# Charrrrrlie/X-as-Supervision

Hardware: AMD Instinct MI355X
Metric: images/sec HM36_Multi_SurS1 256px bs32 (full disc+gen training step) (higher is better)
Workload: dtype f32 (f16x3 split: every fp32 operand as two fp16 pieces, three products; f32 accumulate); 1 GPU; HM36_Multi_SurS1; batch_per_gpu=32, cameras=4, image=256x256, parallelism=dp1, ranks=1, precision=f16x3, dedupe=False, full=False

## Files before the change

include/xas_hip.h:

```cpp
#ifndef XAS_HIP_H
#define XAS_HIP_H

#include <stddef.h>
#include <stdint.h>

#ifdef __cplusplus
extern "C" {
#endif

const char* xas_last_error(void);
enum {
  XAS_TUNE_WGRAD_SPLIT_XCD = 1,
  XAS_TUNE_PLAIN_KLOOP = 32,
  XAS_TUNE_GLOBAL_LOAD = 64,
  XAS_TUNE_WGRAD_GLOBAL_LOAD = 128,
  XAS_TUNE_WGRAD_ALT_ORDER = 8192,
  XAS_TUNE_WGRAD_PLAIN_KLOOP = 524288,
  XAS_TUNE_SLAB_SHIFT = 15,
  XAS_TUNE_SLAB_MASK = 3,
  XAS_TUNE_SLAB_512 = 32768,
  XAS_TUNE_SLAB_128 = 65536,
  XAS_TUNE_SLAB_64 = 98304,
  XAS_TUNE_COL_REDUCE_LEAN = 262144,
  XAS_TUNE_GENERAL_KERNELS = 1 << 22,
  XAS_TUNE_NO_WIDE_TILES = 1 << 23,
  XAS_TUNE_NO_STEM_WGRAD = 1 << 24,
  XAS_TUNE_STEM_FWD_F32 = 1 << 25,
  XAS_TUNE_NO_X6P = 1 << 26,
  XAS_TUNE_X6P_ANY_K = 1 << 27
};
int xas_set_tuning(int flags);
enum { XAS_PREC_F32 = 0, XAS_PREC_BF16 = 1, XAS_PREC_BF16X6 = 2, XAS_PREC_F16X3 = 3 };
#define XAS_AMAX_SUB 32
#define XAS_AMAX_STRIDE 32
#define XAS_AMAX_SLOT_FLOATS (XAS_AMAX_SUB * XAS_AMAX_STRIDE)
enum { XAS_GRAD_IS_X = 0x100 };
int xas_set_precision(int mode);
int xas_get_precision(void);
int xas_abi_version(void);

#define XAS_HEAD_STATS 16
size_t xas_head_workspace_floats(int B, int K, int D);
int xas_head_softargmax_fwd(const float* logits, int B, int K, int D, int num_hypo, int neighbor,
                            float* kps, int64_t* z_idx, float* depth_prob_map, int groups, float* stats,
                            float* partial, void* stream);
int xas_head_softargmax_from_partials(const float* partial, int B, int K, int D, int nchunk, int num_hypo, int neighbor,
                                      float* kps, int64_t* z_idx, float* depth_prob_map, int groups, float* stats,
                                      void* stream);

int xas_head_softargmax_bwd(const float* logits, const float* stats, const int64_t* z_idx,
                            const float* grad_kps, int B, int K, int D, int num_hypo, int neighbor,
                            float* grad_logits, float* coef, void* stream);
int xas_head_softargmax_bwd_amax(const float* logits, const float* stats, const int64_t* z_idx,
                                 const float* grad_kps, int B, int K, int D, int num_hypo, int neighbor,
                                 float* grad_logits, float* coef, float* amax_out, void* stream);

#define XAS_GEO_NORM 1
#define XAS_GEO_MONO 2
#define XAS_GEO_PATCH 4
#define XAS_GEO_IMAGE 8
int xas_patch_to_world_fwd(const float* kps, const float* trans_image, const float* k_mat,
                           const float* pelvis, const float* rot_world, const float* trans_world,
                           int B, int Hy, int K, float image_size, float rect_width, int flags,
                           float* world, void* stream);
int xas_patch_to_world_bwd(const float* kps, const float* grad_world, const float* trans_image,
                           const float* k_mat, const float* pelvis, const float* rot_world,
                           const float* trans_world, int B, int Hy, int K, float image_size,
                           float rect_width, int flags, float* grad_kps, void* stream);

#define XAS_GEO_WORLD 16
int xas_world_to_patch_fwd(const float* pts, const float* pre_rot, float pre_scale, int pelvis_origin,
                           const float* trans_image, const float* k_mat, const float* pelvis,
                           const float* rot_world, const float* trans_world, int B, int Hy, int K,
                           float image_size, float rect_width, int flags, float* out, void* stream);
int xas_world_to_patch_bwd(const float* pts, const float* grad_out, const float* pre_rot, float pre_scale,
                           int pelvis_origin, const float* trans_image, const float* k_mat, const float* pelvis,
                           const float* rot_world, const float* trans_world, int B, int Hy, int K,
                           float image_size, float rect_width, int flags, float* grad_pts, float* grad_pre_rot,
                           void* stream);

int xas_lines_nblk(int S);
int xas_draw_lines_max_fwd(const float* kps, long kp_stride_b, long kp_stride_j, int B, int K,
                           const int* parents, const int* children, int L, unsigned fine_mask,
                           float body_width, int S, float* mask, void* stream);
int xas_draw_lines_max_bwd(const float* kps, long kp_stride_b, long kp_stride_j, int B, int K,
                           const int* parents, const int* children, int L, unsigned fine_mask,
                           float body_width, int S, const float* grad_mask, float* partial,
                           float* grad_kps_xy , void* stream);

typedef struct {
  int N, Hi, Wi, Cin;
  int Cout, R, S;
  int stride, pad;
  int Ho, Wo;
  int mode;
  const float* grad_amax;
  const float* x_amax;
} xas_conv_shape;

int xas_conv_weight_planes(const xas_conv_shape* s, int pass);
int xas_conv_kernel_class(const xas_conv_shape* s, int pass);
int xas_f16_weight_overflow(int reset);
int xas_f16_weight_overflow_peek(unsigned* device_out, void* stream);
size_t xas_split_weight_bytes(long rows, long K, int pieces);
int xas_split_weight(const float* w_packed, void* w_split, long rows, long K, int pieces, void* stream);

int xas_prepare_weights(const void* descs, int n, long blocks, void* stream);

int xas_conv_fwd(const float* x, const float* w_packed, const float* bias, float* y,
                 const xas_conv_shape* s, void* stream);

int xas_conv_fwd_head_chunks(const xas_conv_shape* s, int K, int D);
int xas_conv_fwd_head(const float* x, const float* w_packed, const float* bias, float* y, const xas_conv_shape* s,
                      int K, int D, float* head_partial, void* stream);
size_t xas_conv_fwd_bnstats_workspace_floats(const xas_conv_shape* s, int groups);
int xas_conv_fwd_bnstats(const float* x, const float* w_packed, float* y, const xas_conv_shape* s, int groups,
                         const float* pivot, float* mean, float* var_biased, long out_stride, float* count_out,
                         float* workspace, float* running_mean, float* running_var, float momentum, void* stream);
size_t xas_conv_dgrad_bn_bwd_workspace_floats(const xas_conv_shape* s, int groups);
int xas_conv_dgrad_bn_bwd(const float* dy, const float* w_packed_t, const xas_conv_shape* s, const float* xb,
                          const float* mean, const float* var_biased, const float* gamma, const float* beta, float eps,
                          int groups, double count, float* dz, float* dx, float* sums, float* workspace, float* dbeta_acc,
                          float* dgamma_acc, void* stream);
int xas_conv_dgrad(const float* dy, const float* w_packed_t, float* dx,
                   const xas_conv_shape* s, void* stream);
int xas_conv_dgrad_acc(const float* dy, const float* w_packed_t, float* dx, const xas_conv_shape* shape, void* stream);
int xas_conv_dgrad_acc_masked(const float* dy, const float* w_packed_t, float* dx, const xas_conv_shape* s,
                              const float* dprev, const uint8_t* mask, void* stream);
size_t xas_conv_wgrad_workspace_floats(const xas_conv_shape* s);
int xas_conv_wgrad(const float* x, const float* dy, float* dw_packed, float* workspace,
                   const xas_conv_shape* s, void* stream);
int xas_conv_wgrad_oihw(const float* x, const float* dy, float* dw_oihw, float* workspace,
                        const xas_conv_shape* s, void* stream);
int xas_conv_wgrad_acc(const float* x, const float* dy, float* dw_oihw, float* workspace,
                       const xas_conv_shape* s, void* stream);
int xas_pack_weight(const float* oihw, float* packed, int Cout, int Cin, int R, int S,
                    int transposed, void* stream);
int xas_unpack_weight(const float* packed, float* oihw, int Cout, int Cin, int R, int S,
// ... 128 lines not shown
```

x-as-supervision_amd/csrc/head.hip:

```cpp
#include "common.h"

namespace xas {

struct HeadGeom {
  int B, K, D, HW, W, C4, G, rec;
  int KT, ntile, C4t;
  int R, rh, rw, wshift;
  int P, nchunk;
};

static int pow2_slots(long C4) {
  int gcd = 1;
  while (gcd < 64 && (C4 % (gcd * 2)) == 0) gcd *= 2;
  return 64 / gcd;
}

static bool pow2_policy(int D, int K) {
  if (!(D >= 4 && D <= 64 && (D & (D - 1)) == 0) || (tune_flags() & XAS_TUNE_GENERAL_KERNELS)) return false;
  if (K <= 0) return true;
  const long C4 = (long)K * (D / 4);
  const int R = pow2_slots(C4);
  return R <= D * D && C4 * R <= 1024;
}

// ... 177 lines not shown
  }
  const float S = wave_sum(sd0 + sd1);
  const float pz0 = live0 ? sd0 / S : 0.f, pz1 = live1 ? sd1 / S : 0.f;
  const float X = SX / S, Y = SY / S;
  float* st = stats + ((size_t)b * g.K + k) * XAS_HEAD_STATS;
  if (b % dmap_every == 0) {
    float* dm = depth_prob_map + ((size_t)(b / dmap_every) * g.K + k) * g.D;
    if (live0) dm[d0] = pz0;
    if (live1) dm[d1] = pz1;
  }
  const float fD = (float)g.D;
  const float xn = X / fD * 2.f - 1.f, yn = Y / fD * 2.f - 1.f;
  if (lane == 0) { st[0] = M + __logf(S); st[1] = X; st[2] = Y; }

  if (neighbor == 0) {
    const float Z = wave_sum(pz0 * (float)d0 + pz1 * (float)d1);
    if (lane == 0) {
      float* o = kps + ((size_t)b * g.K + k) * 3;
      o[0] = xn; o[1] = yn; o[2] = Z / fD * 2.f - 1.f;
      st[3] = Z;
      if (z_idx) z_idx[(size_t)b * g.K + k] = 0;
    }
    return;
  }
  float left0 = __shfl_up(pz0, 1, 64), right0 = __shfl_down(pz0, 1, 64);
  float left1 = __shfl_up(pz1, 1, 64), right1 = __shfl_down(pz1, 1, 64);
  const float bin64 = __shfl(pz1, 0, 64), bin63 = __shfl(pz0, 63, 64);
  if (lane == 63) right0 = bin64;
  if (lane == 0) left1 = bin63;
  const bool inner0 = d0 >= 1 && d0 <= g.D - 2, inner1 = d1 <= g.D - 2;
  float score0 = inner0 ? ((pz0 >= left0 && pz0 >= right0) ? pz0 : 0.f) : -1.f;
  float score1 = inner1 ? ((pz1 >= left1 && pz1 >= right1) ? pz1 : 0.f) : -1.f;
  const int r = neighbor / 2;
  for (int h = 0; h < num_hypo; ++h) {
    const float best = wave_max(fmaxf(score0, score1));
    const unsigned long long cand0 = __ballot(score0 == best), cand1 = __ballot(score1 == best);
    const int idx = cand0 ? __ffsll((long long)cand0) - 1 : 64 + __ffsll((long long)cand1) - 1;
    if (d0 == idx) score0 = -2.f;
    if (d1 == idx) score1 = -2.f;
    const bool in0 = live0 && (d0 >= idx - r) && (d0 <= idx + r);
    const bool in1 = live1 && (d1 >= idx - r) && (d1 <= idx + r);
    const float sw = wave_sum((in0 ? pz0 : 0.f) + (in1 ? pz1 : 0.f));
    const float swd = wave_sum((in0 ? pz0 * (float)d0 : 0.f) + (in1 ? pz1 * (float)d1 : 0.f));
    const float Z = swd / sw;
    if (lane == 0) {
      float* o = kps + (((size_t)b * num_hypo + h) * g.K + k) * 3;
      o[0] = xn; o[1] = yn; o[2] = Z / fD * 2.f - 1.f;
      z_idx[((size_t)b * g.K + k) * num_hypo + h] = idx;
      st[3 + h] = Z;
      st[9 + h] = sw;
    }
  }
}

__global__ void head_bwd_coef_kernel(const float* __restrict__ stats, const int64_t* __restrict__ z_idx,
                                     const float* __restrict__ grad_kps, HeadGeom g, int num_hypo, int neighbor,
                                     float* __restrict__ coef) {
  const int b = blockIdx.x / g.K, k = blockIdx.x % g.K;
  const int d = threadIdx.x;
  const float* st = stats + ((size_t)b * g.K + k) * XAS_HEAD_STATS;
  const float fD = (float)g.D;
  float gx = 0.f, gy = 0.f, gz = 0.f, c0 = 0.f;
  const int r = neighbor / 2;
  for (int h = 0; h < num_hypo; ++h) {
    const float* gk = grad_kps + (((size_t)b * num_hypo + h) * g.K + k) * 3;
    gx += gk[0];
    gy += gk[1];
    if (neighbor == 0) {
      const float cz = gk[2] * (2.f / fD);
      gz += cz * (float)d;
      c0 -= cz * st[3];
    } else {
      const int idx = (int)z_idx[((size_t)b * g.K + k) * num_hypo + h];
      if (d >= idx - r && d <= idx + r) gz += gk[2] * (2.f / fD) * ((float)d - st[3 + h]) / st[9 + h];
    }
  }
  const float cx = gx * (2.f / fD), cy = gy * (2.f / fD);
  c0 += -cx * st[1] - cy * st[2];
  float* o = coef + ((size_t)b * g.K + k) * (4 + g.D);
  if (d == 0) { o[0] = cx; o[1] = cy; o[2] = c0; o[3] = st[0]; }
  if (d < g.D) o[4 + d] = gz;
}

template <bool POW2>
__global__ void head_bwd_kernel(const float4* __restrict__ logits, const float* __restrict__ coef, HeadGeom g,
                                float4* __restrict__ grad, float* __restrict__ amax_out) {
  __shared__ unsigned s_amax;
  if (threadIdx.x == 0) s_amax = 0u;
  if (amax_out) __syncthreads();
  float amx = 0.f;
  const int KT = POW2 ? g.K : g.KT, C4t = POW2 ? g.C4 : g.C4t;
  const int tid = threadIdx.x;
  const int c4t = tid % C4t, slot = tid / C4t;
  const int kt = c4t / g.G, dq = c4t % g.G;
  const int bz = POW2 ? 0 : blockIdx.z;
  const int k = bz * KT + kt;
  const int b = blockIdx.y, chunk = blockIdx.x;
  const int pix0 = chunk * g.P;
  const int pend = min(g.P, g.HW - pix0);
  if (POW2 || k < g.K) {
    const float* cf = coef + ((size_t)b * g.K + k) * (4 + g.D);
    const float cx = cf[0], cy = cf[1], c0 = cf[2], lse = cf[3];
    const float4 gz = *reinterpret_cast<const float4*>(cf + 4 + 4 * dq);
    const size_t off = ((size_t)b * g.HW + pix0) * g.C4 + (k * g.G + dq);
    PixelWalk<POW2> walk(g, pix0 + slot);
#pragma unroll 4
    for (int p = slot; p < pend; p += g.R) {
      const float4 v = stream_load(logits + off + (size_t)p * g.C4);
      float fh, fw;
      walk.next(g, pix0 + p, &fh, &fw);
      const float lin = cx * fw + cy * fh + c0;
      float4 o;
      o.x = __expf(v.x - lse) * (lin + gz.x);
      o.y = __expf(v.y - lse) * (lin + gz.y);
      o.z = __expf(v.z - lse) * (lin + gz.z);
      o.w = __expf(v.w - lse) * (lin + gz.w);
      amx = amax4(amx, o);
      stream_store(grad + off + (size_t)p * g.C4, o);
    }
  }
  if (amax_out) {
    if (amx > 0.f) atomicMax(&s_amax, __float_as_uint(amx));
    __syncthreads();
    const unsigned sub = (blockIdx.x + (blockIdx.y + bz * gridDim.y) * gridDim.x) % (unsigned)kAmaxSub;
    if (threadIdx.x == 0 && s_amax) atomicMax(reinterpret_cast<unsigned*>(amax_out + sub * kAmaxStride), s_amax);
  }
}

static int check_modes(const char* who, int D, int num_hypo, int neighbor, const int64_t* z_idx, int B, int groups) {
  XAS_REQUIRE(num_hypo >= 1 && num_hypo <= 6, "%s: num_hypo %d not in [1,6]", who, num_hypo);
  XAS_REQUIRE(neighbor >= 0 && (neighbor > 0 || num_hypo == 1), "%s: single-hypothesis mode needs num_hypo == 1", who);
  XAS_REQUIRE(neighbor == 0 || (z_idx != nullptr && num_hypo <= D - 2), "%s: z_idx required / too many hypotheses", who);
  XAS_REQUIRE(groups >= 1 && B % groups == 0, "%s: B=%d does not split into %d groups", who, B, groups);
  return 0;
}

static int check_grid(const char* who, const HeadGeom& g) {
  XAS_REQUIRE(g.B <= 65535 && g.ntile <= 65535, "%s: B=%d K=%d exceed the launch grid", who, g.B, g.K);
  return 0;
}

static int launch_finalize(const float* partial, const HeadGeom& g, int num_hypo, int neighbor, float* kps, int64_t* z_idx,
                           float* depth_prob_map, int groups, float* stats, void* stream) {
  hipLaunchKernelGGL(head_finalize_kernel, dim3(g.B * g.K), dim3(64), 0, as_stream(stream), partial, g, num_hypo,
                     neighbor, kps, z_idx, depth_prob_map, g.B / groups, stats);
  XAS_LAUNCH_CHECK();
  return 0;
}

}

using namespace xas;

extern "C" size_t xas_head_workspace_floats(int B, int K, int D) {
  HeadGeom g;
  if (make_geom(B, K, D, pow2_policy(D, K), &g)) return 0;
  return (size_t)B * g.nchunk * K * g.rec;
}

extern "C" int xas_head_softargmax_fwd(const float* logits, int B, int K, int D, int num_hypo, int neighbor,
                                       float* kps, int64_t* z_idx, float* depth_prob_map, int groups, float* stats,
                                       float* partial, void* stream) {
  const bool pow2 = pow2_policy(D, K);
  HeadGeom g;
  if (make_geom(B, K, D, pow2, &g)) return 1;
  XAS_REQUIRE(logits && kps && depth_prob_map && stats && partial, "head fwd: null buffer");
  if (check_modes("head fwd", D, num_hypo, neighbor, z_idx, B, groups)) return 1;
  XAS_REQUIRE(((uintptr_t)logits & 15) == 0, "head fwd: logits must be 16-byte aligned");
  const size_t lds = partial_lds_bytes(g, pow2);
  XAS_REQUIRE(lds <= 64 * 1024, "head fwd: LDS %zu too large", lds);
  if (check_grid("head fwd", g)) return 1;
  hipLaunchKernelGGL(pow2 ? head_partial_kernel<true> : head_partial_kernel<false>, dim3(g.nchunk, B, g.ntile),
                     dim3(g.C4t * g.R), lds, as_stream(stream), reinterpret_cast<const float4*>(logits), partial, g);
  XAS_LAUNCH_CHECK();
  return launch_finalize(partial, g, num_hypo, neighbor, kps, z_idx, depth_prob_map, groups, stats, stream);
}

extern "C" int xas_head_softargmax_from_partials(const float* partial, int B, int K, int D, int nchunk, int num_hypo, int neighbor,
                                                 float* kps, int64_t* z_idx, float* depth_prob_map, int groups, float* stats,
                                                 void* stream) {
  HeadGeom g;
  if (make_geom(B, K, D, pow2_policy(D, K), &g)) return 1;
  XAS_REQUIRE(partial && kps && depth_prob_map && stats && nchunk >= 1, "head from partials: null buffer");
  if (check_modes("head from partials", D, num_hypo, neighbor, z_idx, B, groups)) return 1;
  g.nchunk = nchunk;
  return launch_finalize(partial, g, num_hypo, neighbor, kps, z_idx, depth_prob_map, groups, stats, stream);
}

extern "C" int xas_head_softargmax_bwd(const float* logits, const float* stats, const int64_t* z_idx,
                                       const float* grad_kps, int B, int K, int D, int num_hypo, int neighbor,
                                       float* grad_logits, float* coef, void* stream) {
  return xas_head_softargmax_bwd_amax(logits, stats, z_idx, grad_kps, B, K, D, num_hypo, neighbor, grad_logits, coef, nullptr, stream);
}

extern "C" int xas_head_softargmax_bwd_amax(const float* logits, const float* stats, const int64_t* z_idx,
                                            const float* grad_kps, int B, int K, int D, int num_hypo, int neighbor,
                                            float* grad_logits, float* coef, float* amax_out, void* stream) {
  const bool pow2 = pow2_policy(D, K);
  HeadGeom g;
  if (make_geom(B, K, D, pow2, &g)) return 1;
  XAS_REQUIRE(logits && stats && grad_kps && grad_logits && coef, "head bwd: null buffer");
  XAS_REQUIRE(num_hypo >= 1 && num_hypo <= 6, "head bwd: num_hypo %d not in [1,6]", num_hypo);
  XAS_REQUIRE(neighbor == 0 || z_idx != nullptr, "head bwd: z_idx required");
  XAS_REQUIRE((((uintptr_t)logits | (uintptr_t)grad_logits | (uintptr_t)coef) & 15) == 0, "head bwd: 16-byte alignment");
  if (check_grid("head bwd", g)) return 1;
  hipLaunchKernelGGL(head_bwd_coef_kernel, dim3(B * K), dim3(D <= 64 ? 64 : 128), 0, as_stream(stream), stats, z_idx,
                     grad_kps, g, num_hypo, neighbor, coef);
  XAS_LAUNCH_CHECK();
  hipLaunchKernelGGL(pow2 ? head_bwd_kernel<true> : head_bwd_kernel<false>, dim3(g.nchunk, B, g.ntile), dim3(g.C4t * g.R), 0,
                     as_stream(stream), reinterpret_cast<const float4*>(logits), coef, g, reinterpret_cast<float4*>(grad_logits),
                     amax_out);
  XAS_LAUNCH_CHECK();
  return 0;
}
```

x-as-supervision_amd/xas_amd/_lib.py:

```python
import ctypes
import os

import torch

_HERE = os.path.dirname(os.path.abspath(__file__))
LIB_PATH = os.environ.get('XAS_HIP_LIB') or os.path.join(_HERE, 'libxas_hip.so')
_lib = None
ABI_VERSION = 3

_T = {'p': ctypes.c_void_p, 'i': ctypes.c_int, 'l': ctypes.c_long, 'f': ctypes.c_float, 'u': ctypes.c_uint,
      'd': ctypes.c_double, 'z': ctypes.c_size_t}


class ConvShape(ctypes.Structure):
    _fields_ = [(n, ctypes.c_int) for n in ('N', 'Hi', 'Wi', 'Cin', 'Cout', 'R', 'S', 'stride', 'pad', 'Ho', 'Wo', 'mode')] + [
        ('grad_amax', ctypes.c_void_p),
        ('x_amax', ctypes.c_void_p)]


PREC_F32, PREC_BF16, PREC_BF16X6, PREC_F16X3 = 0, 1, 2, 3
PREC_NAMES = {'f32': PREC_F32, 'bf16': PREC_BF16, 'bf16x6': PREC_BF16X6, 'f16x3': PREC_F16X3}

GUARD_FLOATS = 8
GUARD_NORM, GUARD_SCALE, GUARD_SKIP, GUARD_T, GUARD_SKIPPED, GUARD_STEP_SIZE, GUARD_INV_SQRT_BC2, GUARD_NONFINITE = range(8)

TUNE_WGRAD_SPLIT_XCD = 1
TUNE_PLAIN_KLOOP, TUNE_GLOBAL_LOAD, TUNE_WGRAD_GLOBAL_LOAD = 32, 64, 128
TUNE_WGRAD_ALT_ORDER, TUNE_WGRAD_PLAIN_KLOOP = 8192, 524288
TUNE_SLAB_SHIFT, TUNE_SLAB_MASK = 15, 3
TUNE_SLAB_512, TUNE_SLAB_128, TUNE_SLAB_64 = 32768, 65536, 98304
TUNE_COL_REDUCE_LEAN = 262144
TUNE_GENERAL_KERNELS = 1 << 22
TUNE_NO_WIDE_TILES, TUNE_NO_STEM_WGRAD, TUNE_STEM_FWD_F32 = 1 << 23, 1 << 24, 1 << 25
TUNE_NO_X6P, TUNE_X6P_ANY_K = 1 << 26, 1 << 27


SIGNATURES = {
    'xas_abi_version': ('', 'i'),
    'xas_set_tuning': ('i', 'i'),
    'xas_set_precision': ('i', 'i'),
    'xas_get_precision': ('', 'i'),
    'xas_conv_weight_planes': ('si', 'i'),
    'xas_conv_kernel_class': ('si', 'i'),
    'xas_f16_weight_overflow': ('i', 'i'),
    'xas_f16_weight_overflow_peek': ('pp', 'i'),
    'xas_split_weight_bytes': ('lli', 'z'),
    'xas_split_weight': ('ppllip', 'i'),
    'xas_prepare_weights': ('pilp', 'i'),
    'xas_head_workspace_floats': ('iii', 'z'),
    'xas_head_softargmax_fwd': ('piiiiipppippp', 'i'),
    'xas_head_softargmax_bwd': ('ppppiiiiippp', 'i'),
    'xas_head_softargmax_bwd_amax': ('ppppiiiiipppp', 'i'),
    'xas_patch_to_world_fwd': ('ppppppiiiffipp', 'i'),
    'xas_patch_to_world_bwd': ('pppppppiiiffipp', 'i'),
    'xas_world_to_patch_fwd': ('ppfipppppiiiffipp', 'i'),
    'xas_world_to_patch_bwd': ('pppfipppppiiiffippp', 'i'),
    'xas_lines_nblk': ('i', 'i'),
    'xas_draw_lines_max_fwd': ('plliippiufipp', 'i'),
    'xas_draw_lines_max_bwd': ('plliippiufipppp', 'i'),
    'xas_conv_fwd': ('ppppsp', 'i'),
    'xas_conv_fwd_head_chunks': ('sii', 'i'),
    'xas_conv_fwd_head': ('ppppsiipp', 'i'),
    'xas_head_softargmax_from_partials': ('piiiiiipppipp', 'i'),
    'xas_conv_fwd_bnstats_workspace_floats': ('si', 'z'),
    'xas_conv_fwd_bnstats': ('pppsippplppppfp', 'i'),
    'xas_conv_dgrad_bn_bwd_workspace_floats': ('si', 'z'),
    'xas_conv_dgrad_bn_bwd': ('ppspppppfidppppppp', 'i'),
    'xas_conv_dgrad': ('pppsp', 'i'),
    'xas_conv_dgrad_acc': ('pppsp', 'i'),
    'xas_conv_dgrad_acc_masked': ('pppsppp', 'i'),
    'xas_conv_wgrad_workspace_floats': ('s', 'z'),
    'xas_conv_wgrad': ('ppppsp', 'i'),
    'xas_conv_wgrad_oihw': ('ppppsp', 'i'),
    'xas_conv_wgrad_acc': ('ppppsp', 'i'),
    'xas_pack_weight': ('ppiiiiip', 'i'),
    'xas_unpack_weight': ('ppiiiiip', 'i'),
    'xas_bn_workspace_floats': ('lii', 'z'),
    'xas_bn_stats': ('pliipplppppflp', 'i'),
    'xas_bn_stats_from_partials': ('pliilppplppppfp', 'i'),
    'xas_bn_bwd_sums_from_partials': ('pliippppp', 'i'),
    'xas_bn_sync_merge': ('piiilppppfp', 'i'),
    'xas_col_sum': ('plippp', 'i'),
    'xas_col_sum_acc': ('plippp', 'i'),
    'xas_bn_apply': ('ppppppfiliippp', 'i'),
    'xas_bn_apply_amax': ('ppppppfiliipppp', 'i'),
    'xas_abs_max': ('plpp', 'i'),
    'xas_bn_update_running': ('ppppfliip', 'i'),
    'xas_bn_bwd_reduce': ('pppppppfiliipppppp', 'i'),
    'xas_bn_bwd_apply': ('ppppppppfiliidpppp', 'i'),
    'xas_bn_bwd_apply_amax': ('ppppppppfiliidppppp', 'i'),
    'xas_maxpool3x3s2_fwd': ('piiiippp', 'i'),
    'xas_maxpool3x3s2_bwd': ('ppiiiipp', 'i'),
    'xas_upsample2x_fwd': ('piiiipp', 'i'),
    'xas_upsample2x_bwd': ('piiiipp', 'i'),
    'xas_sigmoid_fwd': ('plpp', 'i'),
    'xas_sigmoid_bwd': ('pplpp', 'i'),
    'xas_nchw_to_nhwc': ('piiiipp', 'i'),
    'xas_nhwc_to_nchw': ('piiiipp', 'i'),
    'xas_warp_affine_u8': ('ppppiiipp', 'i'),
    'xas_mask_blur_threshold': ('piipp', 'i'),
    'xas_patch_finish': ('pppppiiippp', 'i'),
    'xas_geodesic_workspace_bytes': ('ii', 'z'),
    'xas_geodesic_weight': ('pppiipppp', 'i'),
    'xas_geodesic_weight_multi': ('ppiipiipppp', 'i'),
    'xas_loss_nblk': ('l', 'i'),
    'xas_mask_loss_fwd': ('pppliPpp'.replace('P', 'p'), 'i'),
    'xas_mask_loss_bwd': ('pppliPppp'.replace('P', 'p'), 'i'),
    'xas_pose_loss_fwd': ('ppiiiifffpp', 'i'),
    'xas_pose_loss_bwd': ('ppiiiifffppppp', 'i'),
    'xas_lsgan_fwd': ('piifppp', 'i'),
    'xas_lsgan_bwd': ('piifpppp', 'i'),
    'xas_graph_aggregate': ('ppiiipp', 'i'),
    'xas_gln_workspace_floats': ('lii', 'z'),
    'xas_gln_fwd': ('ppppliifpppp', 'i'),
    'xas_gln_bwd': ('pppppliifppppp', 'i'),
    'xas_smpl_lbs_fwd': ('ppppppppiiipppp', 'i'),
    'xas_smpl_lbs_bwd_workspace_floats': ('ii', 'z'),
    'xas_smpl_lbs_bwd': ('ppppppppiiippppppp', 'i'),
    'xas_adam_step': ('pppplffffip', 'i'),
    'xas_grad_guard_workspace_bytes': ('l', 'z'),
    'xas_grad_guard': ('plfifffppp', 'i'),
    'xas_adam_step_guarded': ('pppplfffpp', 'i'),
    'xas_eval_select': ('pppiiiifippppp', 'i'),
    'xas_projection_matrix': ('pppipp', 'i'),
    'xas_triangulate_dlt': ('ppiiipp', 'i'),
    'xas_pose_metrics': ('pppiififppppp', 'i'),
}


def load():
    global _lib
    if _lib is not None:
        return _lib
    if not os.path.exists(LIB_PATH):
        raise RuntimeError('libxas_hip.so is missing (%s): run `python __graft_entry__.py` to build the HIP '
# ... 65 lines not shown
```

x-as-supervision_amd/xas_amd/ops_head.py:

```python
import torch

from . import _lib
from ._lib import call, ptr, query

HEAD_STATS = 16
peak_probe = None
GEO_NORM, GEO_MONO, GEO_PATCH = 1, 2, 4
GEO_IMAGE, GEO_WORLD = 8, 16


def _nhwc_storage(logits):
    if logits.dim() != 4:
        raise RuntimeError('logits must be [B, K*D, H, W]')
    if not logits.is_contiguous(memory_format=torch.channels_last):
        logits = logits.contiguous(memory_format=torch.channels_last)
    return logits


def check_patch_size(x, depth_dim, who):
    if x.dim() != 4 or x.shape[-1] != x.shape[-2] or x.shape[-1] != 4 * depth_dim:
        raise RuntimeError('%s(depth_dim=%d) takes square input patches of side 4 * depth_dim = %d, got input %s: build the '
                           'detector with depth_dim = patch size / 4 (a multiple of 4, at most 128: patches up to 512)'
                           % (who, depth_dim, 4 * depth_dim, tuple(x.shape)))


class _SoftArgmax(torch.autograd.Function):
    @staticmethod
    def forward(ctx, logits, num_kp, num_hypo, neighbor, groups):
        from . import ops_nn
        logits_in = logits
        logits_tail = _nhwc_storage(logits)
        logits = ops_nn._full(logits_tail)
        B, C, H, W = logits.shape
        D = C // num_kp
        if not (C == num_kp * D and D == H == W):
            raise RuntimeError('soft-argmax head needs a heat-map cube D == H == W with D a multiple of 4 in [4,128] '
                               '(got C=%d K=%d H=%d W=%d)' % (C, num_kp, H, W))
        dev = logits.device
        kps = torch.empty(B, num_hypo, num_kp, 3, device=dev, dtype=torch.float32)
        z_idx = torch.empty(B, num_kp, num_hypo, device=dev, dtype=torch.int64)
        dmap = torch.empty(groups, num_kp, D, device=dev, dtype=torch.float32)
        stats = torch.empty(B, num_kp, HEAD_STATS, device=dev, dtype=torch.float32)
        pre = getattr(logits_in, '_xas_head', None)
        if pre is not None and pre[2] == logits_in._version and pre[0].shape[0] == B and pre[0].shape[2] == num_kp:
            ops_nn.head_stats['fused'] += 1
            call('xas_head_softargmax_from_partials', ptr(pre[0]), B, num_kp, D, pre[1], num_hypo, neighbor, ptr(kps), ptr(z_idx),
                 ptr(dmap), groups, ptr(stats))
        else:
            ops_nn.head_stats['separate'] += 1
            ws = torch.empty(query('xas_head_workspace_floats', B, num_kp, D), device=dev, dtype=torch.float32)
            call('xas_head_softargmax_fwd', ptr(logits), B, num_kp, D, num_hypo, neighbor, ptr(kps), ptr(z_idx),
                 ptr(dmap), groups, ptr(stats), ptr(ws))
        if peak_probe is not None:
            peak_probe(z_idx.clone())
        s = B - logits_tail.shape[0]
        kps_prefix = kps[:s] if s else kps[:0]
        kps, z_idx_all = (kps[s:], z_idx) if s else (kps, z_idx)
        ctx.save_for_backward(logits_tail, stats[s:] if s else stats, z_idx[s:] if s else z_idx)
        ctx.cfg = (num_kp, D, num_hypo, neighbor)
        ctx.mark_non_differentiable(z_idx_all, dmap, kps_prefix)
        return kps, dmap, z_idx_all, kps_prefix

    @staticmethod
    def backward(ctx, g_kps, _g_dmap, _g_idx, _g_prefix=None):
        logits, stats, z_idx = ctx.saved_tensors
        K, D, Hy, nb = ctx.cfg
        B = logits.shape[0]
        g_kps = g_kps.contiguous()
        grad = torch.empty_like(logits)
        coef = torch.empty(B * K * (4 + D), device=logits.device, dtype=torch.float32)
        from . import ops_nn
        slot = ops_nn.grad_amax_slot(logits.device)
        call('xas_head_softargmax_bwd_amax', ptr(logits), ptr(stats), ptr(z_idx), ptr(g_kps), B, K, D, Hy, nb,
             ptr(grad), ptr(coef), ptr(slot))
        if slot is not None:
            ops_nn.tag_grad_amax(grad, slot)
        return grad, None, None, None, None


def softargmax_multi(logits, num_kp, num_hypo, neighbor_size, groups=1):
    kps, dmap, idx, prefix = _SoftArgmax.apply(logits, num_kp, num_hypo, neighbor_size, groups)
    _last_prefix[0] = prefix
    return kps, (dmap[0] if groups == 1 else dmap), idx


_last_prefix = [None]


def softargmax_single(logits, num_kp, groups=1):
    kps, dmap, _, prefix = _SoftArgmax.apply(logits, num_kp, 1, 0, groups)
    _last_prefix[0] = prefix
    return kps, (dmap[0] if groups == 1 else dmap)


class _PatchToWorld(torch.autograd.Function):
    @staticmethod
    def forward(ctx, kps, ti, km, pv, rw, tw, image_size, rect_width, flags):
        kps = kps.contiguous()
        B, Hy, K, _ = kps.shape
        cams = [t.contiguous().float() for t in (ti, km, pv, rw, tw)]
        world = torch.empty_like(kps)
        call('xas_patch_to_world_fwd', ptr(kps), *[ptr(c) for c in cams], B, Hy, K, float(image_size),
             float(rect_width), flags, ptr(world))
        ctx.save_for_backward(kps, *cams)
        ctx.cfg = (float(image_size), float(rect_width), flags)
        return world

    @staticmethod
    def backward(ctx, gw):
        kps, *cams = ctx.saved_tensors
        B, Hy, K, _ = kps.shape
        S, rect, flags = ctx.cfg
        gk = torch.empty_like(kps)
        call('xas_patch_to_world_bwd', ptr(kps), ptr(gw.contiguous()), *[ptr(c) for c in cams], B, Hy, K, S, rect,
             flags, ptr(gk))
        return (gk,) + (None,) * 8


def patch_to_world(kps, trans_image, k_mat, pelvis, rot_world, trans_world, image_size=256, rect_width=2000.0,
                   is_norm=True, mono=False, patch=True):
    squeeze = kps.dim() == 3
    if squeeze:
        kps = kps.unsqueeze(1)
    flags = (GEO_NORM if is_norm else 0) | (GEO_MONO if mono else 0) | (GEO_PATCH if patch else 0)
    out = _PatchToWorld.apply(kps, trans_image, k_mat, pelvis, rot_world, trans_world, image_size, rect_width, flags)
    return out.squeeze(1) if squeeze else out


class _WorldToPatch(torch.autograd.Function):
    @staticmethod
    def forward(ctx, pts, pre_rot, ti, km, pv, rw, tw, pre_scale, pelvis_origin, image_size, rect_width, flags):
        pts = pts.contiguous()
        B, Hy, K, _ = pts.shape
        rot = pre_rot.contiguous() if pre_rot is not None else None
        cams = [t.contiguous().float() for t in (ti, km, pv, rw, tw)]
        out = torch.empty_like(pts)
        call('xas_world_to_patch_fwd', ptr(pts), ptr(rot), float(pre_scale), int(pelvis_origin), *[ptr(c) for c in cams],
             B, Hy, K, float(image_size), float(rect_width), flags, ptr(out))
        ctx.save_for_backward(pts, *cams, *(() if rot is None else (rot,)))
        ctx.cfg = (float(pre_scale), int(pelvis_origin), float(image_size), float(rect_width), flags)
        return out

    @staticmethod
    def backward(ctx, go):
        pts, ti, km, pv, rw, tw, *rot = ctx.saved_tensors
        rot = rot[0] if rot else None
        B, Hy, K, _ = pts.shape
        scale, origin, S, rect, flags = ctx.cfg
        gp = torch.empty_like(pts)
        grot = torch.empty_like(rot) if rot is not None else None
        call('xas_world_to_patch_bwd', ptr(pts), ptr(go.contiguous()), ptr(rot), scale, origin, ptr(ti), ptr(km), ptr(pv),
             ptr(rw), ptr(tw), B, Hy, K, S, rect, flags, ptr(gp), ptr(grot))
        return (gp, grot) + (None,) * 10


def world_to_patch(points, params, mode, is_norm=True, RECT_WIDTH=2000, pre_rot=None, pre_scale=1.0, pelvis_origin=False,
                   stop_at_image=False, stop_at_world=False):
# ... 60 lines not shown
```

x-as-supervision_amd/xas_amd/ops_nn.py:

```python
import os

import torch
import torch.distributed as dist

from . import _lib
from . import streams
from ._lib import ConvShape, call, ptr, query

CL = torch.channels_last
_weights_epoch = [0]

_groups = [1]

_prefix = [0, 0]


class bn_groups:
    def __init__(self, groups, prefix_groups=0, images_per_group=0):
        self.groups = int(groups)
        self.prefix = [int(prefix_groups) * int(images_per_group), int(prefix_groups)]
        if self.prefix[1] and not (0 < self.prefix[1] < self.groups and images_per_group > 0):
            raise RuntimeError('bn_groups: the no-grad prefix must be a proper, non-empty subset of the groups')

    def __enter__(self):
# ... 84 lines not shown
    if _side['dirty'] and _side['stream'] is not None:
        ev = torch.cuda.Event()
        ev.record(_side['stream'])
        return ev
    return None


_uses = {'on': False, 'pending': {}, 'hook': None}


def track_grad_uses(on=True):
    _uses['on'] = bool(on)
    _uses['pending'].clear()


def note_use(p):
    if _uses['on'] and p is not None:
        k = p.data_ptr()
        _uses['pending'][k] = _uses['pending'].get(k, 0) + 1


def grad_ready(p):
    if not _uses['on']:
        return
    k = p.data_ptr()
    if k not in _uses['pending']:
        return
    left = _uses['pending'][k] - 1
    if left > 0:
        _uses['pending'][k] = left
        return
    del _uses['pending'][k]
    if _uses['hook'] is not None:
        _uses['hook'](p)


def forget_uses(keys):
    for k in keys:
        _uses['pending'].pop(k, None)


def _wgrad_into_grad(x, dy, shp, weight):
    g = weight.grad
    if g is None or not g.is_contiguous() or g.dtype != torch.float32 or not g.is_cuda:
        return False
    if not _side['enabled']:
        ws = torch.empty(max(1, query('xas_conv_wgrad_workspace_floats', shp)), device=x.device, dtype=torch.float32)
        call('xas_conv_wgrad_acc', ptr(x), ptr(dy), ptr(g), ptr(ws), shp)
        grad_ready(weight)
        return True
    main, side = torch.cuda.current_stream(), side_stream()
    side.wait_stream(main)
    with torch.cuda.stream(side):
        ws = torch.empty(max(1, query('xas_conv_wgrad_workspace_floats', shp)), device=x.device, dtype=torch.float32)
        call('xas_conv_wgrad_acc', ptr(x), ptr(dy), ptr(g), ptr(ws), shp)
    _keep_for_side(x, dy)
    _side['dirty'] = True
    grad_ready(weight)
    return True


BIAS_ON_SIDE = os.environ.get('XAS_BIAS_SIDE', '0') == '1'


def _bias_into_grad(dy, M, C, bias, force=False):
    g = bias.grad
    if (not (BIAS_ON_SIDE or force or not _side['enabled']) or g is None or not g.is_contiguous() or g.dtype != torch.float32 or C % 4
            or g.data_ptr() % 16 or not g.is_cuda):
        return False
    if not _side['enabled']:
        ws = torch.empty(query('xas_bn_workspace_floats', M, C, 1), device=dy.device, dtype=torch.float32)
        call('xas_col_sum_acc', ptr(dy), M, C, ptr(g), ptr(ws))
        grad_ready(bias)
        return True
    main, side = torch.cuda.current_stream(), side_stream()
    side.wait_stream(main)
    with torch.cuda.stream(side):
        ws = torch.empty(query('xas_bn_workspace_floats', M, C, 1), device=dy.device, dtype=torch.float32)
        call('xas_col_sum_acc', ptr(dy), M, C, ptr(g), ptr(ws))
    _keep_for_side(dy)
    _side['dirty'] = True
    grad_ready(bias)
    return True


def to_cl(x):
    if x.dim() != 4:
        raise RuntimeError('expected a 4-D activation tensor')
    return x if x.is_contiguous(memory_format=CL) else x.contiguous(memory_format=CL)


def empty_cl(n, c, h, w, like):
    return torch.empty((n, c, h, w), device=like.device, dtype=torch.float32, memory_format=CL)


def from_nchw(x):
    if x.is_contiguous(memory_format=CL):
        return x
    x = x.contiguous()
    n, c, h, w = x.shape
    y = empty_cl(n, c, h, w, x)
    call('xas_nchw_to_nhwc', ptr(x), n, c, h, w, ptr(y))
    return y


def stack_nchw(tensors):
    t0 = tensors[0]
    if (len(tensors) == 1 or t0.dim() != 4 or not t0.is_cuda or t0.shape[1] == 1
            or any(t.requires_grad or (t.is_contiguous(memory_format=CL) and t.shape[1] > 1) for t in tensors)):
        return torch.cat(list(tensors), dim=0) if len(tensors) > 1 else t0
    n, c, h, w = t0.shape
    y = empty_cl(n * len(tensors), c, h, w, t0)
    for g, t in enumerate(tensors):
        t = t.contiguous()
        call('xas_nchw_to_nhwc', ptr(t), n, c, h, w, ptr(y[g * n:(g + 1) * n]))
    return y


def _shape(n, hi, wi, cin, cout, r, s, stride, pad, ho, wo, mode=0):
    return ConvShape(n, hi, wi, cin, cout, r, s, stride, pad, ho, wo, mode)


MODE_F32 = 1 + _lib.PREC_F32
GRAD_IS_X = 0x100


_amax = {'arena': None, 'next': 0, 'retired': [], 'epoch': 0}
_AMAX_SLOTS = 2048
AMAX_SLOT_FLOATS = 1024
GRAD_F16 = os.environ.get('XAS_GRAD_F16', '1') == '1'
amax_stats = {'abs_max': 0}


def reset_grad_amax():
    if _amax['arena'] is not None and _amax['next'] > 0:
        _amax['arena'][:_amax['next'] * AMAX_SLOT_FLOATS].zero_()
    _amax['next'] = 0
    _amax['retired'] = []
    _amax['epoch'] += 1


def _amax_slot(device):
    a = _amax['arena']
    if a is None or a.device != device or _amax['next'] >= _AMAX_SLOTS:
        if a is not None:
            _amax['retired'] = (_amax['retired'] + [a])[-4:]
        a = _amax['arena'] = torch.zeros(_AMAX_SLOTS * AMAX_SLOT_FLOATS, device=device, dtype=torch.float32)
        _amax['next'] = 0
    i = _amax['next']
    _amax['next'] = i + 1
    return a[i * AMAX_SLOT_FLOATS:(i + 1) * AMAX_SLOT_FLOATS]


def amax_slot_from_value(v):
    s = torch.zeros(AMAX_SLOT_FLOATS, device=v.device, dtype=torch.float32)
    s[0] = v.reshape(())
    return s


def f16x3_on():
    return GRAD_F16 and query('xas_get_precision') == _lib.PREC_F16X3


def grad_amax_slot(device):
    if not f16x3_on():
        return None
# ... 97 lines not shown
        box = getattr(w, '_xas_epoch', _weights_epoch)
        key = (w.data_ptr(), w._version, box[0])
        if key != self.key:
            self.key, self.packed = key, {}

    def get(self, w, transposed, shp=None, planes=None):
        self._fresh(w)
        if planes is None:
            planes = query('xas_conv_weight_planes', shp, int(transposed)) if shp is not None else 0
        k = (transposed, planes)
        if k in self.packed:
            return self.packed[k]
        if (transposed, 0) not in self.packed:
            co, ci, r, s = w.shape
            if not transposed and r == 1 and s == 1 and w.is_contiguous() and w.data_ptr() % 16 == 0:
                self.packed[(transposed, 0)] = w.detach().view(-1)
            else:
                p = torch.empty(w.numel(), device=w.device, dtype=torch.float32)
                call('xas_pack_weight', ptr(w.detach().contiguous()), ptr(p), co, ci, r, s, int(transposed))
                self.packed[(transposed, 0)] = p
        if planes:
            src = self.packed[(transposed, 0)]
            rows = w.shape[1] if transposed else w.shape[0]
            kk = src.numel() // rows
            sp = torch.empty(query('xas_split_weight_bytes', rows, kk, planes), device=w.device, dtype=torch.uint8)
            call('xas_split_weight', ptr(src), ptr(sp), rows, kk, planes)
            self.packed[k] = sp
        return self.packed[k]


def _col_sum(t2d_ptr_tensor, M, C):
    out = torch.empty(C, device=t2d_ptr_tensor.device, dtype=torch.float32)
    ws = torch.empty(query('xas_bn_workspace_floats', M, C, 1), device=out.device, dtype=torch.float32)
    call('xas_col_sum', ptr(t2d_ptr_tensor), M, C, ptr(out), ptr(ws))
    return out


def _bias_grad(dy, M, C):
    if C % 4 == 0:
        return _col_sum(dy, M, C)
    return dy.reshape(M, C).sum(0)


def _wgrad(x, dy, shp, w_shape, transposed=False):
    co, ci, r, s = shp.Cout, shp.Cin, shp.R, shp.S
    ws = torch.empty(max(1, query('xas_conv_wgrad_workspace_floats', shp)), device=x.device, dtype=torch.float32)
    dw = torch.empty(w_shape, device=x.device, dtype=torch.float32)
    call('xas_conv_wgrad_oihw', ptr(x), ptr(dy), ptr(dw), ptr(ws), shp)
    return dw


HEAD_IN_EPILOGUE = os.environ.get('XAS_HEAD_IN_EPILOGUE', '1') == '1'
head_stats = {'fused': 0, 'separate': 0}


class _Conv2d(torch.autograd.Function):
    @staticmethod
    def forward(ctx, x, weight, bias, stride, pad, cache, head_kd=None):
        x = to_cl(x)
        n, ci, hi, wi = x.shape
        co, ci2, r, s = weight.shape
        if ci != ci2:
            raise RuntimeError('conv2d: input has %d channels, weight expects %d' % (ci, ci2))
        ho, wo = (hi + 2 * pad - r) // stride + 1, (wi + 2 * pad - s) // stride + 1
        shp, x_slot = with_act_amax(_shape(n, hi, wi, ci, co, r, s, stride, pad, ho, wo), x)
        xf = _full(x)
        yf = empty_cl(xf.shape[0], co, ho, wo, x)
        shp_f = _with_n(shp, xf.shape[0])
        chunks = query('xas_conv_fwd_head_chunks', shp_f, head_kd[0], head_kd[1]) if (head_kd and HEAD_IN_EPILOGUE and x.is_cuda) else 0
        if chunks:
            rec = torch.empty(xf.shape[0], chunks, head_kd[0], 3 + head_kd[1], device=x.device, dtype=torch.float32)
            call('xas_conv_fwd_head', ptr(xf), ptr(cache.get(weight, 0, shp_f)), ptr(bias), ptr(yf), shp_f, head_kd[0], head_kd[1], ptr(rec))
        else:
            call('xas_conv_fwd', ptr(xf), ptr(cache.get(weight, 0, shp_f)), ptr(bias), ptr(yf), shp_f)
        y = _tail(yf)
        if chunks:
            y._xas_head = (rec, chunks, y._version)
        ctx.save_for_backward(x, weight, *([bias] if bias is not None else []))
        ctx.shp, ctx.cache, ctx.has_bias, ctx.x_slot = shp, cache, bias is not None, x_slot
        if ctx.needs_input_grad[1]:
            note_use(weight)
        if bias is not None and ctx.needs_input_grad[2]:
            note_use(bias)
        return y

    @staticmethod
    def backward(ctx, dy):
        x, weight, *rest = ctx.saved_tensors
        shp = with_grad_amax(ctx.shp, dy, ctx.x_slot)
        dy = to_cl(dy)
        dx = dw = db = None
        if ctx.needs_input_grad[0]:
            dx = torch.empty_like(x)
            call('xas_conv_dgrad', ptr(dy), ptr(ctx.cache.get(weight, 1, shp)), ptr(dx), shp)
        if ctx.needs_input_grad[1] and not _wgrad_into_grad(x, dy, shp, weight):
            dw = _wgrad(x, dy, shp, weight.shape)
        if ctx.has_bias and ctx.needs_input_grad[2]:
            M = shp.N * shp.Ho * shp.Wo
            if not _bias_into_grad(dy, M, shp.Cout, rest[0]):
                db = _bias_grad(dy, M, shp.Cout)
        return dx, dw, db, None, None, None, None


def conv2d(x, weight, bias, stride, pad, cache, head_kd=None):
    return _Conv2d.apply(x, weight, bias, stride, pad, cache, head_kd)


def _conv_forward(x, weight, stride, pad, cache):
    n, ci, hi, wi = x.shape
    co, ci2, r, s = weight.shape
    if ci != ci2:
        raise RuntimeError('conv2d: input has %d channels, weight expects %d' % (ci, ci2))
    ho, wo = (hi + 2 * pad - r) // stride + 1, (wi + 2 * pad - s) // stride + 1
    shp, _ = with_act_amax(_shape(n, hi, wi, ci, co, r, s, stride, pad, ho, wo), x)
    xf = _full(x)
    yf = empty_cl(xf.shape[0], co, ho, wo, x)
    shp_f = _with_n(shp, xf.shape[0])
    call('xas_conv_fwd', ptr(xf), ptr(cache.get(weight, 0, shp_f)), None, ptr(yf), shp_f)
    return _tail(yf), shp


FUSE_CONV_STATS = os.environ.get('XAS_CONV_STATS', '1') == '1'


def _conv_bn_forward(x, conv, bn, residual, group):
    weight = conv.weight
    if not (FUSE_CONV_STATS and bn.training):
        y, shp = _conv_forward(x, weight, conv.stride, conv.padding, conv._cache)
        out, sv, cf = _bn_forward(y, bn.weight, bn.bias, bn.running_mean, bn.running_var, residual, bn.training,
                                  bn.momentum, bn.eps, bn.act, group)
        return out, sv, cf, shp
    n, ci, hi, wi = x.shape
    co, ci2, r, s = weight.shape
    if ci != ci2:
        raise RuntimeError('conv2d: input has %d channels, weight expects %d' % (ci, ci2))
    stride, pad = conv.stride, conv.padding
    ho, wo = (hi + 2 * pad - r) // stride + 1, (wi + 2 * pad - s) // stride + 1
    shp, _ = with_act_amax(_shape(n, hi, wi, ci, co, r, s, stride, pad, ho, wo), x)
    xf = _full(x)
    shp_f = _with_n(shp, xf.shape[0])
    yf = empty_cl(xf.shape[0], co, ho, wo, x)
    y = _tail(yf)
    wp = conv._cache.get(weight, 0, shp_f)
    G = _groups[0]
    pivot = None

    def stats(mean_p, var_p, out_stride, count_p, rm_p, rv_p, momentum):
        ws = torch.empty(query('xas_conv_fwd_bnstats_workspace_floats', shp_f, G), device=x.device, dtype=torch.float32)
        call('xas_conv_fwd_bnstats', ptr(xf), ptr(wp), ptr(yf), shp_f, G, ptr(pivot), mean_p, var_p, out_stride, count_p,
             ptr(ws), rm_p, rv_p, float(momentum))

    out, sv, cf = _bn_forward(y, bn.weight, bn.bias, bn.running_mean, bn.running_var, residual, True, bn.momentum,
                              bn.eps, bn.act, group, stats_fn=stats)
    return out, sv, cf, shp


FUSE_DGRAD_BN = os.environ.get('XAS_DGRAD_BN', '0') == '1'


def _bn_bwd_fusable(cfg):
    M, c, eps, act, count, group, training, has_res, xfree, yfree, G, masked = cfg
    return training and group is None and act == ACT_RELU and not has_res and yfree and not masked


def _conv_dgrad_bn_bwd(dy, conv, shp, saved, cfg, bn, want_param_grads):
    xb, _, mean, var = saved
    M, c, eps, act, count, group, training, has_res, xfree, yfree, G, masked = cfg
    dy = to_cl(dy)
    dev = xb.device
    gamma, beta = bn.weight, bn.bias
    sums = torch.empty(G, 2, c, device=dev, dtype=torch.float32)
    ws = torch.empty(query('xas_conv_dgrad_bn_bwd_workspace_floats', shp, G), device=dev, dtype=torch.float32)
    gg, gb = gamma.grad, beta.grad
    direct = (want_param_grads and gg is not None and gb is not None and gg.is_contiguous() and gb.is_contiguous()
              and gg.dtype == torch.float32 and gb.dtype == torch.float32)
    dz = torch.empty_like(xb)
    dx = torch.empty_like(xb)
    shp_n = _with_ptrs(shp, None, None)
    call('xas_conv_dgrad_bn_bwd', ptr(dy), ptr(conv._cache.get(conv.weight, 1, shp_n)), shp_n, ptr(xb), ptr(mean), ptr(var),
         ptr(gamma), ptr(beta), float(eps), G, float(count), ptr(dz), ptr(dx), ptr(sums), ptr(ws),
         ptr(gb) if direct else None, ptr(gg) if direct else None)
    if direct:
# ... 620 lines not shown
```

Measured before the change: 2091 images/s.

## Fuse head conv bias-gradient column sums into softargmax backward kernel

```diff
diff --git a/include/xas_hip.h b/include/xas_hip.h
--- a/include/xas_hip.h
+++ b/include/xas_hip.h
@@ -54,6 +54,11 @@
 int xas_head_softargmax_bwd_amax(const float* logits, const float* stats, const int64_t* z_idx,
                                  const float* grad_kps, int B, int K, int D, int num_hypo, int neighbor,
                                  float* grad_logits, float* coef, float* amax_out, void* stream);
+size_t xas_head_bwd_colsum_workspace_floats(int B, int K, int D);
+int xas_head_softargmax_bwd_amax_colsum(const float* logits, const float* stats, const int64_t* z_idx,
+                                        const float* grad_kps, int B, int K, int D, int num_hypo, int neighbor,
+                                        float* grad_logits, float* coef, float* amax_out, float* bias_grad,
+                                        float* workspace, void* stream);
 
 #define XAS_GEO_NORM 1
 #define XAS_GEO_MONO 2
diff --git a/x-as-supervision_amd/csrc/head.hip b/x-as-supervision_amd/csrc/head.hip
--- a/x-as-supervision_amd/csrc/head.hip
+++ b/x-as-supervision_amd/csrc/head.hip
@@ -283,13 +283,20 @@
   if (d < g.D) o[4 + d] = gz;
 }
 
-template <bool POW2>
+__device__ __forceinline__ void comp_add(float& s, float& c, float v) {
+  const float y = v - c, t = s + y;
+  c = (t - s) - y;
+  s = t;
+}
+
+template <bool POW2, bool COLSUM = false>
 __global__ void head_bwd_kernel(const float4* __restrict__ logits, const float* __restrict__ coef, HeadGeom g,
-                                float4* __restrict__ grad, float* __restrict__ amax_out) {
+                                float4* __restrict__ grad, float* __restrict__ amax_out, float* __restrict__ colsum) {
   __shared__ unsigned s_amax;
   if (threadIdx.x == 0) s_amax = 0u;
   if (amax_out) __syncthreads();
   float amx = 0.f;
+  float4 cs = make_float4(0.f, 0.f, 0.f, 0.f), cc = cs;
   const int KT = POW2 ? g.K : g.KT, C4t = POW2 ? g.C4 : g.C4t;
   const int tid = threadIdx.x;
   const int c4t = tid % C4t, slot = tid / C4t;
@@ -317,7 +324,21 @@
       o.z = __expf(v.z - lse) * (lin + gz.z);
       o.w = __expf(v.w - lse) * (lin + gz.w);
       amx = amax4(amx, o);
+      if constexpr (COLSUM) { comp_add(cs.x, cc.x, o.x); comp_add(cs.y, cc.y, o.y); comp_add(cs.z, cc.z, o.z); comp_add(cs.w, cc.w, o.w); }
       stream_store(grad + off + (size_t)p * g.C4, o);
+    }
+  }
+  if constexpr (COLSUM) {
+    extern __shared__ float4 s_cs[];
+    s_cs[tid] = cs;
+    __syncthreads();
+    if (slot == 0 && (POW2 || k < g.K)) {
+      float4 t = s_cs[c4t], tc = make_float4(0.f, 0.f, 0.f, 0.f);
+      for (int s = 1; s < g.R; ++s) {
+        const float4 u = s_cs[s * C4t + c4t];
+        comp_add(t.x, tc.x, u.x); comp_add(t.y, tc.y, u.y); comp_add(t.z, tc.z, u.z); comp_add(t.w, tc.w, u.w);
+      }
+      reinterpret_cast<float4*>(colsum + ((size_t)b * g.nchunk + chunk) * ((size_t)g.C4 * 4))[k * g.G + dq] = t;
     }
   }
   if (amax_out) {
@@ -388,6 +409,29 @@
   return launch_finalize(partial, g, num_hypo, neighbor, kps, z_idx, depth_prob_map, groups, stats, stream);
 }
 
+static int launch_bwd(const float* logits, const float* stats, const int64_t* z_idx, const float* grad_kps, int B, int K, int D,
+                      int num_hypo, int neighbor, float* grad_logits, float* coef, float* amax_out, float* colsum, HeadGeom* geom,
+                      void* stream) {
+  const bool pow2 = pow2_policy(D, K);
+  HeadGeom& g = *geom;
+  if (make_geom(B, K, D, pow2, &g)) return 1;
+  XAS_REQUIRE(logits && stats && grad_kps && grad_logits && coef, "head bwd: null buffer");
+  XAS_REQUIRE(num_hypo >= 1 && num_hypo <= 6, "head bwd: num_hypo %d not in [1,6]", num_hypo);
+  XAS_REQUIRE(neighbor == 0 || z_idx != nullptr, "head bwd: z_idx required");
+  XAS_REQUIRE((((uintptr_t)logits | (uintptr_t)grad_logits | (uintptr_t)coef | (uintptr_t)colsum) & 15) == 0, "head bwd: 16-byte alignment");
+  if (check_grid("head bwd", g)) return 1;
+  hipLaunchKernelGGL(head_bwd_coef_kernel, dim3(B * K), dim3(D <= 64 ? 64 : 128), 0, as_stream(stream), stats, z_idx,
+                     grad_kps, g, num_hypo, neighbor, coef);
+  XAS_LAUNCH_CHECK();
+  const auto k = colsum ? (pow2 ? head_bwd_kernel<true, true> : head_bwd_kernel<false, true>)
+                        : (pow2 ? head_bwd_kernel<true> : head_bwd_kernel<false>);
+  const size_t lds = colsum ? (size_t)g.C4t * g.R * sizeof(float4) : 0;
+  hipLaunchKernelGGL(k, dim3(g.nchunk, B, g.ntile), dim3(g.C4t * g.R), lds, as_stream(stream),
+                     reinterpret_cast<const float4*>(logits), coef, g, reinterpret_cast<float4*>(grad_logits), amax_out, colsum);
+  XAS_LAUNCH_CHECK();
+  return 0;
+}
+
 extern "C" int xas_head_softargmax_bwd(const float* logits, const float* stats, const int64_t* z_idx,
                                        const float* grad_kps, int B, int K, int D, int num_hypo, int neighbor,
                                        float* grad_logits, float* coef, void* stream) {
@@ -397,20 +441,25 @@
 extern "C" int xas_head_softargmax_bwd_amax(const float* logits, const float* stats, const int64_t* z_idx,
                                             const float* grad_kps, int B, int K, int D, int num_hypo, int neighbor,
                                             float* grad_logits, float* coef, float* amax_out, void* stream) {
-  const bool pow2 = pow2_policy(D, K);
-  HeadGeom g;
-  if (make_geom(B, K, D, pow2, &g)) return 1;
-  XAS_REQUIRE(logits && stats && grad_kps && grad_logits && coef, "head bwd: null buffer");
-  XAS_REQUIRE(num_hypo >= 1 && num_hypo <= 6, "head bwd: num_hypo %d not in [1,6]", num_hypo);
-  XAS_REQUIRE(neighbor == 0 || z_idx != nullptr, "head bwd: z_idx required");
-  XAS_REQUIRE((((uintptr_t)logits | (uintptr_t)grad_logits | (uintptr_t)coef) & 15) == 0, "head bwd: 16-byte alignment");
-  if (check_grid("head bwd", g)) return 1;
-  hipLaunchKernelGGL(head_bwd_coef_kernel, dim3(B * K), dim3(D <= 64 ? 64 : 128), 0, as_stream(stream), stats, z_idx,
-                     grad_kps, g, num_hypo, neighbor, coef);
-  XAS_LAUNCH_CHECK();
-  hipLaunchKernelGGL(pow2 ? head_bwd_kernel<true> : head_bwd_kernel<false>, dim3(g.nchunk, B, g.ntile), dim3(g.C4t * g.R), 0,
-                     as_stream(stream), reinterpret_cast<const float4*>(logits), coef, g, reinterpret_cast<float4*>(grad_logits),
-                     amax_out);
-  XAS_LAUNCH_CHECK();
-  return 0;
-}
+  HeadGeom g;
+  return launch_bwd(logits, stats, z_idx, grad_kps, B, K, D, num_hypo, neighbor, grad_logits, coef, amax_out, nullptr, &g, stream);
+}
+
+extern "C" size_t xas_head_bwd_colsum_workspace_floats(int B, int K, int D) {
+  HeadGeom g;
+  if (make_geom(B, K, D, pow2_policy(D, K), &g)) return 0;
+  const long rows = (long)B * g.nchunk;
+  return (size_t)rows * K * D + xas_bn_workspace_floats(rows, K * D, 1);
+}
+
+extern "C" int xas_head_softargmax_bwd_amax_colsum(const float* logits, const float* stats, const int64_t* z_idx,
+                                                   const float* grad_kps, int B, int K, int D, int num_hypo, int neighbor,
+                                                   float* grad_logits, float* coef, float* amax_out, float* bias_grad,
+                                                   float* workspace, void* stream) {
+  XAS_REQUIRE(bias_grad && workspace, "head bwd: the column-sum form needs bias_grad and its workspace");
+  HeadGeom g;
+  if (launch_bwd(logits, stats, z_idx, grad_kps, B, K, D, num_hypo, neighbor, grad_logits, coef, amax_out, workspace, &g, stream))
+    return 1;
+  const long rows = (long)B * g.nchunk;
+  return xas_col_sum_acc(workspace, rows, K * D, bias_grad, workspace + (size_t)rows * K * D, stream);
+}
diff --git a/x-as-supervision_amd/xas_amd/_lib.py b/x-as-supervision_amd/xas_amd/_lib.py
--- a/x-as-supervision_amd/xas_amd/_lib.py
+++ b/x-as-supervision_amd/xas_amd/_lib.py
@@ -51,6 +51,8 @@
     'xas_head_softargmax_fwd': ('piiiiipppippp', 'i'),
     'xas_head_softargmax_bwd': ('ppppiiiiippp', 'i'),
     'xas_head_softargmax_bwd_amax': ('ppppiiiiipppp', 'i'),
+    'xas_head_bwd_colsum_workspace_floats': ('iii', 'z'),
+    'xas_head_softargmax_bwd_amax_colsum': ('ppppiiiiipppppp', 'i'),
     'xas_patch_to_world_fwd': ('ppppppiiiffipp', 'i'),
     'xas_patch_to_world_bwd': ('pppppppiiiffipp', 'i'),
     'xas_world_to_patch_fwd': ('ppfipppppiiiffipp', 'i'),
diff --git a/x-as-supervision_amd/xas_amd/ops_head.py b/x-as-supervision_amd/xas_amd/ops_head.py
--- a/x-as-supervision_amd/xas_amd/ops_head.py
+++ b/x-as-supervision_amd/xas_amd/ops_head.py
@@ -58,6 +58,7 @@
         kps, z_idx_all = (kps[s:], z_idx) if s else (kps, z_idx)
         ctx.save_for_backward(logits_tail, stats[s:] if s else stats, z_idx[s:] if s else z_idx)
         ctx.cfg = (num_kp, D, num_hypo, neighbor)
+        ctx.colsum = ops_nn.wants_colsum(logits_in)
         ctx.mark_non_differentiable(z_idx_all, dmap, kps_prefix)
         return kps, dmap, z_idx_all, kps_prefix
 
@@ -71,8 +72,15 @@
         coef = torch.empty(B * K * (4 + D), device=logits.device, dtype=torch.float32)
         from . import ops_nn
         slot = ops_nn.grad_amax_slot(logits.device)
-        call('xas_head_softargmax_bwd_amax', ptr(logits), ptr(stats), ptr(z_idx), ptr(g_kps), B, K, D, Hy, nb,
-             ptr(grad), ptr(coef), ptr(slot))
+        if ctx.colsum:
+            sums = torch.zeros(K * D, device=logits.device, dtype=torch.float32)
+            ws = torch.empty(query('xas_head_bwd_colsum_workspace_floats', B, K, D), device=logits.device, dtype=torch.float32)
+            call('xas_head_softargmax_bwd_amax_colsum', ptr(logits), ptr(stats), ptr(z_idx), ptr(g_kps), B, K, D, Hy, nb,
+                 ptr(grad), ptr(coef), ptr(slot), ptr(sums), ptr(ws))
+            ops_nn.offer_colsum(grad, sums)
+        else:
+            call('xas_head_softargmax_bwd_amax', ptr(logits), ptr(stats), ptr(z_idx), ptr(g_kps), B, K, D, Hy, nb,
+                 ptr(grad), ptr(coef), ptr(slot))
         if slot is not None:
             ops_nn.tag_grad_amax(grad, slot)
         return grad, None, None, None, None
diff --git a/x-as-supervision_amd/xas_amd/ops_nn.py b/x-as-supervision_amd/xas_amd/ops_nn.py
--- a/x-as-supervision_amd/xas_amd/ops_nn.py
+++ b/x-as-supervision_amd/xas_amd/ops_nn.py
@@ -190,6 +190,25 @@
     _side['dirty'] = True
     grad_ready(bias)
     return True
+
+
+FUSED_BIAS_SUMS = os.environ.get('XAS_FUSED_BIAS_SUMS', '1') == '1'
+bias_sum_stats = {'fused': 0, 'separate': 0}
+
+
+def wants_colsum(t):
+    return FUSED_BIAS_SUMS and getattr(t, '_xas_wants_colsum', None) == t._version
+
+
+def offer_colsum(grad, sums):
+    grad._xas_colsum = (sums, grad._version)
+
+
+def take_colsum(dy, C):
+    tag = getattr(dy, '_xas_colsum', None)
+    if tag is None or tag[1] != dy._version or tag[0].numel() != C:
+        return None
+    return tag[0]
 
 
 def to_cl(x):
@@ -453,12 +472,15 @@
             note_use(weight)
         if bias is not None and ctx.needs_input_grad[2]:
             note_use(bias)
+            if FUSED_BIAS_SUMS and co % 4 == 0 and x.is_cuda:
+                y._xas_wants_colsum = y._version
         return y
 
     @staticmethod
     def backward(ctx, dy):
         x, weight, *rest = ctx.saved_tensors
         shp = with_grad_amax(ctx.shp, dy, ctx.x_slot)
+        sums = take_colsum(dy, shp.Cout) if ctx.has_bias else None
         dy = to_cl(dy)
         dx = dw = db = None
         if ctx.needs_input_grad[0]:
@@ -468,7 +490,11 @@
             dw = _wgrad(x, dy, shp, weight.shape)
         if ctx.has_bias and ctx.needs_input_grad[2]:
             M = shp.N * shp.Ho * shp.Wo
-            if not _bias_into_grad(dy, M, shp.Cout, rest[0]):
+            bias_sum_stats['separate' if sums is None else 'fused'] += 1
+            if sums is not None:
+                if not _bias_into_grad(sums, 1, shp.Cout, rest[0]):
+                    db = sums
+            elif not _bias_into_grad(dy, M, shp.Cout, rest[0]):
                 db = _bias_grad(dy, M, shp.Cout)
         return dx, dw, db, None, None, None, None
 
```

Result: no change. 2103 images/s, median of 6 (+0.6%).
